# facebookresearch/videoseal

Measured on AMD Instinct MI355X. Metric: frames/sec embed+extract 256-bit @768x768, higher is better.
Workload: dtype f32 (2 x f16 operand split, 3 products on v_mfma_f32_32x32x16_f16, fp32 accumulate); 1 GPU; videoseal_1.0 256-bit, 32 frames 768x768 per GPU, image mode (embedder on every frame, full-res JND), embed + detect; card=videoseal_1.0, weights=random-init (seeded), no checkpoint offline, batch_per_gpu=32, mode=image

## Files before the change

videoseal_amd/csrc/net_ops.hip:

```cpp
#include <algorithm>
#include <cstdlib>
#include <cstring>

#include "conv_common.h"
#include "upconv_gather.h"

namespace {

__global__ __launch_bounds__(256) void layernorm_act_kernel(const float* __restrict__ x, int64_t rows, int C, int64_t ld,
                                                            const float* __restrict__ w, const float* __restrict__ b,
                                                            float eps, int act, float* __restrict__ out, int64_t out_ld) {
  const int lane = threadIdx.x & 63;
  const int64_t row = (int64_t)blockIdx.x * 4 + (threadIdx.x >> 6);
  if (row >= rows) return;
  const float* xr = x + row * ld;
  float s = 0.f;
  for (int c = lane; c < C; c += 64) s += xr[c];
  const float mean = wave_sum(s) / (float)C;
  float v = 0.f;
  for (int c = lane; c < C; c += 64) {
    const float dlt = xr[c] - mean;
    v += dlt * dlt;
  }
  const float var = wave_sum(v) / (float)C;
// ... 359 lines not shown
    for (int k = 0; k < LIN; ++k) {
      rin[k] = f32x4{0.f, 0.f, 0.f, 0.f};
      if (g_off[k] >= 0) rin[k] = *reinterpret_cast<const f32x4*>(xb + g_off[k] + c0);
    }
#pragma unroll
    for (int k = 0; k < LWT; ++k) {
      const int i = tid + k * NT;
      const int cg = i % N4, t = i / N4;
      if (i < NWT) rwt[k] = *reinterpret_cast<const f32x4*>((t < 49 ? wdw + (int64_t)t * ld : bdw) + c0 + cg * 4);
    }
  };
  const int nch = (int)ld / CCH;
  fetch(0);
  for (int ch = 0; ch < nch; ++ch) {
    const int c0 = ch * CCH;
#pragma unroll
    for (int k = 0; k < LIN; ++k)
      if (l_off[k] >= 0) *reinterpret_cast<f32x4*>(s_in + l_off[k]) = rin[k];
#pragma unroll
    for (int k = 0; k < LWT; ++k) {
      const int i = tid + k * NT;
      if (i < NWT) *reinterpret_cast<f32x4*>(s_w + (i / N4) * CCH + (i % N4) * 4) = rwt[k];
    }
    __syncthreads();
    if (ch + 1 < nch) fetch(c0 + CCH);
#ifdef VS_DWT_ABL
    if (!(VS_DWT_ABL & 2))
#endif
    for (int it = tid; it < ITEMS; it += NT) {
      const int cg = it % N4, rs = it / N4;
      const int sx = rs % SPR, r = rs / SPR;
      f32x4 acc[4];
      const f32x4 bv = *reinterpret_cast<const f32x4*>(s_w + 49 * CCH + cg * 4);
#pragma unroll
      for (int p = 0; p < 4; ++p) acc[p] = bv;
#pragma unroll
      for (int ky = 0; ky < 7; ++ky) {
        const float* row = s_in + ((r + ky) * IW + sx * 4) * CP + cg * 4;
        f32x4 in[10];
#pragma unroll
        for (int j = 0; j < 10; ++j) in[j] = *reinterpret_cast<const f32x4*>(row + j * CP);
#pragma unroll
        for (int kx = 0; kx < 7; ++kx) {
          const f32x4 wv = *reinterpret_cast<const f32x4*>(s_w + (ky * 7 + kx) * CCH + cg * 4);
#pragma unroll
          for (int p = 0; p < 4; ++p) acc[p] += in[p + kx] * wv;
        }
      }
#pragma unroll
      for (int p = 0; p < 4; ++p) *reinterpret_cast<f32x4*>(s_out + (int64_t)(r * TW + sx * 4 + p) * (ld + 4) + c0 + cg * 4) = acc[p];
    }
    __syncthreads();
  }
#ifdef VS_DWT_ABL
  if (VS_DWT_ABL & 1) return;
#endif
  ln_rows_from_lds<NT>(s_out, (int)ld + 4, TH * TW, C, lnw, lnb, eps, (int)out_ld, [&](int p) -> float* {
    const int gy = y0 + p / TW, gx = x0 + p % TW;
    return (gy < H && gx < W) ? out + (((int64_t)b * H + gy) * W + gx) * out_ld : nullptr;
  }, pl, wb_sep ? s_wbs : (2 * C <= (TH + 6) * (TW + 6) * CP) ? s_in : nullptr, wb_sep != 0);
}

template <int TH, int TW, int CCH, int NT>
static int launch_dwconv_tiled(const float* x, int B, int H, int W, int C, int64_t ld, const float* wdw, const float* bdw, const float* lnw,
                               const float* lnb, float eps, float* out, int64_t out_ld, hipStream_t st, PlanesOut pl = PlanesOut{0, 0, 1.f, 0}) {
  size_t smem = sizeof(float) * ((size_t)(TH + 6) * (TW + 6) * (CCH + 4) + 50 * CCH + (size_t)TH * TW * (ld + 4));
  if (smem > 160 * 1024 || ld % CCH != 0 || (int64_t)H * W * ld >= (1ll << 31)) return VS_ERR_UNSUPPORTED;
  const int wb_sep = smem + 2 * sizeof(float) * (size_t)C <= 160 * 1024;
  if (wb_sep) smem += 2 * sizeof(float) * (size_t)C;
  auto kern = dwconv7_ln_tiled_kernel<TH, TW, CCH, NT>;
  static size_t attr_set = 0;
  if (smem > 64 * 1024 && smem > attr_set) {
    (void)hipFuncSetAttribute((const void*)kern, hipFuncAttributeMaxDynamicSharedMemorySize, 160 * 1024);
    attr_set = 160 * 1024;
  }
  const int tiles_x = (W + TW - 1) / TW, tiles_y = (H + TH - 1) / TH;
  const int64_t nblk = (int64_t)B * tiles_x * tiles_y;
  if (nblk >= (1 << 30)) return VS_ERR_UNSUPPORTED;
  hipLaunchKernelGGL(kern, dim3((unsigned)((nblk + 7) / 8 * 8)), dim3(NT), smem, st, x, H, W, C, ld, wdw, bdw, lnw, lnb, eps, out, out_ld,
                     tiles_x, tiles_y, (int)nblk, pl, wb_sep);
  return vs_launch_status();
}

constexpr int GRN_ROWS = 64;
__global__ __launch_bounds__(256) void grn_partial_kernel(const float* __restrict__ h, int HW, int C, int64_t ld,
                                                          float* __restrict__ partial, int B) {
  const int c = blockIdx.x * 256 + threadIdx.x;
  const int chunk = blockIdx.y, b = blockIdx.z;
  if (c >= C) return;
  const int r0 = chunk * GRN_ROWS, r1 = min(HW, r0 + GRN_ROWS);
  const float* p = h + ((int64_t)b * HW + r0) * ld + c;
  float s = 0.f;
  for (int r = r0; r < r1; ++r, p += ld) s += (*p) * (*p);
  partial[((int64_t)chunk * B + b) * C + c] = s;
}
template <int NB, int KB>
__global__ __launch_bounds__(1024) void grn_finish_kernel(const float* __restrict__ partial, int nchunk, int B, int C,
                                                          const float* __restrict__ gamma, float* __restrict__ scale,
                                                          int64_t sld, int frame_major) {
  __shared__ float grp[NB][4][256];
  __shared__ float red[256];
  const int b = blockIdx.x;
  const int cl = threadIdx.x & 255, kg = threadIdx.x >> 8;
  const int kper = (nchunk + 3) / 4;
  const int k0 = kg * kper, k1 = min(nchunk, k0 + kper);
  float local = 0.f;
  for (int cb0 = 0; cb0 < C; cb0 += 256 * NB) {
    float s[NB];
#pragma unroll
    for (int j = 0; j < NB; ++j) s[j] = 0.f;
    const int64_t kstride = frame_major ? (int64_t)C : (int64_t)B * C;
    const float* rowp = frame_major ? partial + ((int64_t)b * nchunk + k0) * C : partial + ((int64_t)k0 * B + b) * C;
    int k = k0;
    for (; k + KB <= k1; k += KB, rowp += KB * kstride) {
      float v[KB][NB];
#pragma unroll
      for (int q = 0; q < KB; ++q)
#pragma unroll
        for (int j = 0; j < NB; ++j) {
          const int c = cb0 + j * 256 + cl;
          v[q][j] = c < C ? rowp[q * kstride + c] : 0.f;
        }
#pragma unroll
      for (int q = 0; q < KB; ++q)
#pragma unroll
        for (int j = 0; j < NB; ++j) s[j] += v[q][j];
    }
    if constexpr (KB > 4) {
      for (; k + 4 <= k1; k += 4, rowp += 4 * kstride) {
        float v[4][NB];
#pragma unroll
        for (int q = 0; q < 4; ++q)
#pragma unroll
          for (int j = 0; j < NB; ++j) {
            const int c = cb0 + j * 256 + cl;
            v[q][j] = c < C ? rowp[q * kstride + c] : 0.f;
          }
#pragma unroll
        for (int q = 0; q < 4; ++q)
#pragma unroll
          for (int j = 0; j < NB; ++j) s[j] += v[q][j];
      }
    }
    for (; k < k1; ++k, rowp += kstride) {
#pragma unroll
      for (int j = 0; j < NB; ++j) {
        const int c = cb0 + j * 256 + cl;
        if (c < C) s[j] += rowp[c];
      }
    }
#pragma unroll
    for (int j = 0; j < NB; ++j) grp[j][kg][cl] = s[j];
    __syncthreads();
    if (kg == 0) {
#pragma unroll
      for (int j = 0; j < NB; ++j) {
        const int c = cb0 + j * 256 + cl;
        if (c < C) {
          const float gx = sqrtf(((grp[j][0][cl] + grp[j][1][cl]) + grp[j][2][cl]) + grp[j][3][cl]);
          scale[(int64_t)b * sld + c] = gx;
          local += gx;
        }
      }
    }
    __syncthreads();
  }
// ... 589 lines not shown
  const int qd = threadIdx.x & 3;
  const int64_t npix = (int64_t)B * Ho * Wo;
  const int64_t pix = (int64_t)blockIdx.x * 64 + (threadIdx.x >> 2);
  const bool live = pix < npix;
  const int64_t pc = live ? pix : npix - 1;
  const int ox = (int)(pc % Wo);
  const int64_t t = pc / Wo;
  const int oy = (int)(t % Ho);
  const int64_t b = t / Ho;
  const float* xp = x + ((b * H + (int64_t)oy * stride) * W + (int64_t)ox * stride) * 4;
  f32x4 acc[Q4];
#pragma unroll
  for (int j = 0; j < Q4; ++j) acc[j] = *reinterpret_cast<const f32x4*>(bias + qd * CQ + 4 * j);
#pragma unroll
  for (int ky = 0; ky < 4; ++ky) {
    f32x4 in[4];
#pragma unroll
    for (int kx = 0; kx < 4; ++kx) in[kx] = *reinterpret_cast<const f32x4*>(xp + ((int64_t)ky * W + kx) * 4);
#pragma unroll
    for (int kx = 0; kx < 4; ++kx)
#pragma unroll
      for (int c = 0; c < 3; ++c) {
        const float v = in[kx][c];
        const float* wr = s_w + (ky * 12 + kx * 3 + c) * CO + qd * CQ;
#pragma unroll
        for (int j = 0; j < Q4; ++j) {
          const f32x4 wv = *reinterpret_cast<const f32x4*>(wr + 4 * j);
#pragma unroll
          for (int e = 0; e < 4; ++e) acc[j][e] = __builtin_fmaf(v, wv[e], acc[j][e]);
        }
      }
  }
  float sm = 0.f;
#pragma unroll
  for (int j = 0; j < Q4; ++j)
#pragma unroll
    for (int e = 0; e < 4; ++e) sm += acc[j][e];
  sm += __shfl_xor(sm, 1, 64);
  sm += __shfl_xor(sm, 2, 64);
  const float mean = sm / (float)CO;
  float qv = 0.f;
#pragma unroll
  for (int j = 0; j < Q4; ++j)
#pragma unroll
    for (int e = 0; e < 4; ++e) { const float dlt = acc[j][e] - mean; qv += dlt * dlt; }
  qv += __shfl_xor(qv, 1, 64);
  qv += __shfl_xor(qv, 2, 64);
  const float den = sqrtf(qv / (float)CO + eps);
  if (!live) return;
  float* orow = out + pix * out_ld + qd * CQ;
#pragma unroll
  for (int j = 0; j < Q4; ++j) {
    const f32x4 wv = *reinterpret_cast<const f32x4*>(lnw + qd * CQ + 4 * j), bv = *reinterpret_cast<const f32x4*>(lnb + qd * CQ + 4 * j);
    f32x4 o;
#pragma unroll
    for (int e = 0; e < 4; ++e) o[e] = wv[e] * ((acc[j][e] - mean) / den) + bv[e];
    *reinterpret_cast<f32x4*>(orow + 4 * j) = o;
  }
}

extern "C" int vs_stem_conv_ln(const float* x, int B, int H, int W, int stride, const float* wt, const float* bias, const float* lnw, const float* lnb,
                               float eps, int CO, float* out, int64_t out_ld, void* stream) {
  VS_REQUIRE(x && wt && bias && lnw && lnb && out && B > 0 && H >= 4 && W >= 4 && (stride == 4 || stride == 2));
  if ((CO != 64 && CO != 96 && CO != 128) || out_ld != CO ||
      (((uintptr_t)x | (uintptr_t)wt | (uintptr_t)bias | (uintptr_t)lnw | (uintptr_t)lnb | (uintptr_t)out) & 15) != 0)
    return VS_ERR_UNSUPPORTED;
  const int Ho = (H - 4) / stride + 1, Wo = (W - 4) / stride + 1;
  const int64_t npix = (int64_t)B * Ho * Wo;
  if (npix >= (1LL << 31) * 16) return VS_ERR_UNSUPPORTED;
  const dim3 grid((unsigned)cdiv64(npix, 64));
  hipStream_t st = (hipStream_t)stream;
  if (CO == 96) hipLaunchKernelGGL(stem_conv_ln_kernel<96>, grid, dim3(256), 0, st, x, B, H, W, Ho, Wo, stride, wt, bias, lnw, lnb, eps, out, out_ld);
  else if (CO == 64) hipLaunchKernelGGL(stem_conv_ln_kernel<64>, grid, dim3(256), 0, st, x, B, H, W, Ho, Wo, stride, wt, bias, lnw, lnb, eps, out, out_ld);
  else hipLaunchKernelGGL(stem_conv_ln_kernel<128>, grid, dim3(256), 0, st, x, B, H, W, Ho, Wo, stride, wt, bias, lnw, lnb, eps, out, out_ld);
  return vs_launch_status();
}

static int dwconv7_ln_any(const float* x, int B, int H, int W, int C, int64_t ld, const float* wdw, const float* bdw,
                          const float* lnw, const float* lnb, float eps, float* out, int64_t out_ld, void* stream, PlanesOut pl) {
  VS_REQUIRE(x && wdw && bdw && lnw && lnb && out && B > 0 && H > 0 && W > 0 && C > 0);
  VS_REQUIRE(ld % 4 == 0 && ld >= C && (pl.cstride || (out_ld >= C && out_ld % 4 == 0)));
  const int force = vs_debug_get(VS_DBG_DWCONV) - 1;
  {
    const int64_t hw = (int64_t)H * W;
    int cfg = 0;
    if (force >= 0) cfg = force;
    else if (hw >= 4096) cfg = 5;
    else if (hw >= 1024) cfg = 3;
    else if (hw >= 256) cfg = 6;
    int rc = VS_ERR_UNSUPPORTED;
    if (cfg == 1) rc = launch_dwconv_tiled<8, 8, 48, 256>(x, B, H, W, C, ld, wdw, bdw, lnw, lnb, eps, out, out_ld, (hipStream_t)stream, pl);
    else if (cfg == 2) rc = launch_dwconv_tiled<4, 8, 64, 128>(x, B, H, W, C, ld, wdw, bdw, lnw, lnb, eps, out, out_ld, (hipStream_t)stream, pl);
    else if (cfg == 3) rc = launch_dwconv_tiled<8, 16, 32, 256>(x, B, H, W, C, ld, wdw, bdw, lnw, lnb, eps, out, out_ld, (hipStream_t)stream, pl);
    else if (cfg == 4) rc = launch_dwconv_tiled<4, 16, 64, 256>(x, B, H, W, C, ld, wdw, bdw, lnw, lnb, eps, out, out_ld, (hipStream_t)stream, pl);
    else if (cfg == 5) rc = launch_dwconv_tiled<4, 16, 48, 256>(x, B, H, W, C, ld, wdw, bdw, lnw, lnb, eps, out, out_ld, (hipStream_t)stream, pl);
    else if (cfg == 6) rc = launch_dwconv_tiled<4, 8, 128, 256>(x, B, H, W, C, ld, wdw, bdw, lnw, lnb, eps, out, out_ld, (hipStream_t)stream, pl);
    else if (cfg == 7) rc = launch_dwconv_tiled<4, 4, 128, 128>(x, B, H, W, C, ld, wdw, bdw, lnw, lnb, eps, out, out_ld, (hipStream_t)stream, pl);
    else if (cfg == 8) rc = launch_dwconv_tiled<4, 4, 64, 128>(x, B, H, W, C, ld, wdw, bdw, lnw, lnb, eps, out, out_ld, (hipStream_t)stream, pl);
    else if (cfg == 9) rc = launch_dwconv_tiled<4, 4, 32, 128>(x, B, H, W, C, ld, wdw, bdw, lnw, lnb, eps, out, out_ld, (hipStream_t)stream, pl);
    else if (cfg == 10) rc = launch_dwconv_tiled<2, 8, 64, 128>(x, B, H, W, C, ld, wdw, bdw, lnw, lnb, eps, out, out_ld, (hipStream_t)stream, pl);
    if (rc == VS_ERR_UNSUPPORTED && force < 0 && cfg == 3)
      rc = launch_dwconv_tiled<4, 16, 48, 256>(x, B, H, W, C, ld, wdw, bdw, lnw, lnb, eps, out, out_ld, (hipStream_t)stream, pl);
    if (rc != VS_ERR_UNSUPPORTED) return rc;
  }
  const int C4 = (int)(ld / 4);
  int NS = 256 / C4;
  if (NS < 1) NS = 1;
  const int spr = (W + 3) / 4;
  const int dbg_rows = vs_debug_get(VS_DBG_DWCONV_ROWS);
  const bool two = dbg_rows ? dbg_rows == 2 : (NS == 1 && H >= 2 && (int64_t)B * ((H + 1) / 2) * spr >= vs_num_cus());
  const int R = two ? 2 : 1;
  const int64_t nstrips = (int64_t)B * ((H + R - 1) / R) * spr;
  const size_t smem = ((size_t)NS * 4 * R * (ld + 4) + 2 * (size_t)C) * sizeof(float);
  if (smem > 160 * 1024) return VS_ERR_UNSUPPORTED;
  if (two) {
    if (smem > 64 * 1024)
      (void)hipFuncSetAttribute((const void*)dwconv7_ln_kernel<2>, hipFuncAttributeMaxDynamicSharedMemorySize, (int)smem);
    hipLaunchKernelGGL(dwconv7_ln_kernel<2>, dim3((unsigned)cdiv64(nstrips, NS)), dim3(256), smem, (hipStream_t)stream, x, B, H, W,
                       C, ld, wdw, bdw, lnw, lnb, eps, out, out_ld, NS, spr, nstrips, pl);
    return vs_launch_status();
  }
  if (smem > 64 * 1024)
    (void)hipFuncSetAttribute((const void*)dwconv7_ln_kernel<1>, hipFuncAttributeMaxDynamicSharedMemorySize, (int)smem);
  hipLaunchKernelGGL(dwconv7_ln_kernel<1>, dim3((unsigned)cdiv64(nstrips, NS)), dim3(256), smem, (hipStream_t)stream, x, B, H, W,
                     C, ld, wdw, bdw, lnw, lnb, eps, out, out_ld, NS, spr, nstrips, pl);
  return vs_launch_status();
}

extern "C" int vs_dwconv7_ln(const float* x, int B, int H, int W, int C, int64_t ld, const float* wdw, const float* bdw,
                             const float* lnw, const float* lnb, float eps, float* out, int64_t out_ld, void* stream) {
  return dwconv7_ln_any(x, B, H, W, C, ld, wdw, bdw, lnw, lnb, eps, out, out_ld, stream, PlanesOut{0, 0, 1.f, 0});
}
extern "C" int vs_dwconv7_ln_planes(const float* x, int B, int H, int W, int C, int64_t ld, const float* wdw, const float* bdw,
                                    const float* lnw, const float* lnb, float eps, float a_mul, int planes_C, void* planes, void* stream) {
  VS_REQUIRE(planes && a_mul > 0.f && ((uintptr_t)planes & 15) == 0 && planes_C >= C && planes_C % 16 == 0);
  const int64_t rows = (int64_t)B * H * W, cstride = rows * 32;
  return dwconv7_ln_any(x, B, H, W, C, ld, wdw, bdw, lnw, lnb, eps, static_cast<float*>(planes), 8, stream,
                        PlanesOut{cstride, (int64_t)(planes_C / 16) * cstride, a_mul, planes_C});
}

extern "C" int vs_grn_scale(const float* h, int B, int HW, int C, int64_t ld, const float* gamma, float* partial,
                            float* scale, void* stream) {
  VS_REQUIRE(h && gamma && partial && scale && B > 0 && HW > 0 && C > 0 && ld >= C);
  const int nchunk = (HW + GRN_ROWS - 1) / GRN_ROWS;
  hipLaunchKernelGGL(grn_partial_kernel, dim3((unsigned)((C + 255) / 256), (unsigned)nchunk, (unsigned)B), dim3(256), 0,
                     (hipStream_t)stream, h, HW, C, ld, partial, B);
  if (C <= 512) hipLaunchKernelGGL((grn_finish_kernel<2, 16>), dim3((unsigned)B), dim3(1024), 0, (hipStream_t)stream, partial, nchunk, B, C, gamma,
                     scale, ld, 0);
  else if (C <= 1024) hipLaunchKernelGGL((grn_finish_kernel<4, 8>), dim3((unsigned)B), dim3(1024), 0, (hipStream_t)stream, partial, nchunk, B, C, gamma,
                     scale, ld, 0);
  else hipLaunchKernelGGL((grn_finish_kernel<8, 4>), dim3((unsigned)B), dim3(1024), 0, (hipStream_t)stream, partial, nchunk, B, C, gamma,
                     scale, ld, 0);
  return vs_launch_status();
}

__global__ __launch_bounds__(256) void grn_apply_kernel(float* __restrict__ h, int64_t rows, int HW, int C, int64_t ld,
                                                        const float* __restrict__ scale, int64_t sld, const float* __restrict__ beta) {
  const int C4 = (C + 3) >> 2;
  const int64_t idx = (int64_t)blockIdx.x * 256 + threadIdx.x;
  if (idx >= rows * C4) return;
  const int64_t m = idx / C4;
  const int c = (int)(idx - m * C4) * 4;
  const int b = (int)(m / HW);
  f32x4 v = *reinterpret_cast<f32x4*>(h + m * ld + c);
  const f32x4 s = *reinterpret_cast<const f32x4*>(scale + (int64_t)b * sld + c);
  const f32x4 sh = *reinterpret_cast<const f32x4*>(beta + c);
  const f32x4 o = v * s + sh;
#pragma unroll
  for (int e = 0; e < 4; ++e) v[e] = c + e < C ? o[e] : v[e];
  *reinterpret_cast<f32x4*>(h + m * ld + c) = v;
}

extern "C" int vs_grn_apply(float* h, int B, int HW, int C, int64_t ld, const float* scale, int64_t scale_ld, const float* beta,
                            void* stream) {
  VS_REQUIRE(h && scale && beta && B > 0 && HW > 0 && C > 0 && ld >= C && (ld & 3) == 0 && (scale_ld & 3) == 0 && scale_ld >= ((C + 3) & ~3));
  const int64_t rows = (int64_t)B * HW, items = rows * ((C + 3) >> 2);
  hipLaunchKernelGGL(grn_apply_kernel, dim3((unsigned)cdiv64(items, 256)), dim3(256), 0, (hipStream_t)stream, h, rows, HW, C, ld, scale,
                     scale_ld, beta);
  return vs_launch_status();
}

extern "C" int vs_grn_scale_from_partials(const float* partial, int B, int HW, int C, const float* gamma, float* scale,
                                          int64_t scale_ld, void* stream) {
  VS_REQUIRE(partial && gamma && scale && B > 0 && HW > 0 && HW % 32 == 0 && C > 0 && scale_ld >= C);
  if (C <= 512) hipLaunchKernelGGL((grn_finish_kernel<2, 16>), dim3((unsigned)B), dim3(1024), 0, (hipStream_t)stream, partial, HW / 32, B, C, gamma,
// ... 239 lines not shown
```

videoseal_amd/csrc/vs_common.h:

```cpp
#pragma once
#include <hip/hip_runtime.h>
#include <stdint.h>
#include <stdlib.h>
#include <string.h>

#include "videoseal_hip.h"

typedef float f32x4 __attribute__((ext_vector_type(4)));
typedef float f32x16 __attribute__((ext_vector_type(16)));

#define VS_REQUIRE(cond)                  \
  do {                                    \
    if (!(cond)) return VS_ERR_BAD_ARG;   \
  } while (0)

static inline int vs_launch_status() { return hipGetLastError() == hipSuccess ? VS_OK : VS_ERR_LAUNCH; }

static inline int64_t cdiv64(int64_t a, int64_t b) { return (a + b - 1) / b; }

static inline vs_yuv420_surface_t vs_nv12_surface(const void* base, int H, int64_t pitch, int64_t frame_stride) {
  vs_yuv420_surface_t s{};
  unsigned char* p = static_cast<unsigned char*>(const_cast<void*>(base));
  s.plane[0] = p;
  s.plane[1] = p + (int64_t)H * pitch;
  s.pitch[0] = s.pitch[1] = pitch;
  s.frame_stride[0] = s.frame_stride[1] = frame_stride;
  s.depth = 8;
  return s;
}

#define VS_DBG_ANY (-0x7fffffff - 1)
#define VS_DBG_KEYS(X)                                                                                                                              \
  X(RESIZE_FORM, "VIDEOSEAL_RESIZE", "tile=1", 0, 1, "vs_resize_pre(_nv12): 1 = the 32 x 8 tile kernel")                                            \
  X(RESIZE_STRIP, "VS_RESIZE_STRIP", nullptr, 0, 2, "vs_resize_pre(_nv12): strip height in output rows (the variable from 2, the key from 1)")      \
  X(TAIL_STRIP, "VS_TAIL_STRIP", nullptr, 0, 4, "vs_embed_tail(_nv12): strip height in rows, rounded up to 4 (from 4)")                             \
  X(JPEG_FORM, "VIDEOSEAL_JPEG", "scalar=1", 0, 1, "JPEG round trip: 1 = the one-pixel-per-lane kernels")                                           \
  X(CROP_RESIZE_FORM, "VIDEOSEAL_CROP_RESIZE", "tile=1", 0, 1, "Crop -> Resize -> colour: 1 = the 32 x 8 tile kernel")                              \
  X(TO_PLANES_FORM, nullptr, nullptr, 0, 1, "vs_to_planes_affine: 1 = one row per wave")                                                            \
  X(DWCONV_ROWS, "VS_DWCONV_ROWS", nullptr, 0, VS_DBG_ANY, "one-row depthwise kernel: 2 = two output rows per strip, any other value = one")        \
  X(LN_FORM, "VIDEOSEAL_LN", "wave=1", 0, 1, "vs_layernorm_act: 1 = one wave per row")                                                              \
  X(SPLITK_EPI, "VS_SPLITK_EPI", "s*=1", 0, 1, "K-slice epilogue: 1 = the first kernel, one load in flight per thread (VS_SPLITK_EPI=scalar)")      \
  X(UPCONV_FORM, nullptr, nullptr, 0, 1, "vs_upconv_gather_ln and phase 3 of vs_upconv_fused: 1 = per-pixel gather instead of 2 x 2 blocks")        \
  X(TAIL_FORM, "VIDEOSEAL_TAIL", "v1=1,sep=2,keep=3", 0, 1, "vs_embed_tail: the numbers of vs_tail_desc_t::variant (which overrides it per call)")  \
  X(VIT_ATTN, "VS_VIT_ATTN", "valu=1", 0, 1, "vs_vit_attention: 1 = the vector kernel on the matrix-core shapes too")                               \
  X(WGRAD, "VS_WGRAD", "mfma=1,fma=2", 0, 1, "vs_gemm_wgrad: 1 = the fp32 matrix-core kernel, 2 = the fp32 vector kernel, everywhere")              \
  X(DWCONV, "VS_DWCONV", nullptr, 1, 1, "depthwise 7 x 7 + LayerNorm: 1 + configuration (1 = the one-row kernel, 2.. = tiled; VS_DWCONV=0 -> 1)")    \
  X(GEMM_GRID, "VS_GEMM_GRID", nullptr, 0, 1, "wave-specialised 1 x 1 GEMM: workgroups of the persistent grid instead of one per CU")               \
  X(GEMM_PL_RASTER, "VS_GEMM_PL_RASTER", "0*=1", 0, 1, "planes GEMMs: 1 = row-major tile order instead of the XCD-grouped one (the variable: 0)")    \
  X(CNX_PIPE, "VS_CNX_PIPE", nullptr, 1, 1, "fused ConvNeXt block: 1 = the serial cnx_block_kernel (VS_CNX_PIPE=0), any other value = the pipeline") \
  X(CNX_ABL, "VS_CNX_ABL", nullptr, 0, VS_DBG_ANY, "fused ConvNeXt block: ablation bits (builds with VS_CNX_ABLATION only)")                        \
  X(UPCONV_ABL, "VS_UPCONV_ABL", nullptr, 0, VS_DBG_ANY, "vs_upconv_fused: ablation bits")                                                          \
  X(STEM_FUSED, "VIDEOSEAL_STEM_FUSED", "1*=1", 0, 1, "vs_model_detect: 1 = stem conv + LayerNorm in one kernel")                                   \
  X(ARITH, "VIDEOSEAL_CONV", "f16x2=2,bf16x3=3", 0, 2, "default vs_conv_desc_t::arith of the model-level entry points")
#define VS_DBG_ENUM(name, env, words, bias, min, doc) VS_DBG_##name,
enum { VS_DBG_KEYS(VS_DBG_ENUM) VS_DBG_COUNT };
#undef VS_DBG_ENUM
static_assert(VS_DBG_RESIZE_FORM == 0 && VS_DBG_UPCONV_FORM == 9 && VS_DBG_ARITH == 20 && VS_DBG_COUNT == 21, "development switch keys keep their numbers");

#define VS_DEFAULT_ARITH 2
static inline int vs_default_arith() {
  const int a = vs_debug_get(VS_DBG_ARITH);
  return a == 2 || a == 3 ? a : VS_DEFAULT_ARITH;
}

static inline int vs_max_lds_bytes() {
  static const int n = [] {
    int dev = 0, v = 0;
    if (hipGetDevice(&dev) != hipSuccess || hipDeviceGetAttribute(&v, hipDeviceAttributeMaxSharedMemoryPerBlock, dev) != hipSuccess || v <= 0) v = 64 * 1024;
    return v;
  }();
  return n;
}

static inline int vs_num_cus() {
  static const int n = [] {
    int dev = 0, v = 0;
    if (hipGetDevice(&dev) != hipSuccess || hipDeviceGetAttribute(&v, hipDeviceAttributeMultiprocessorCount, dev) != hipSuccess || v <= 0) v = 256;
    return v;
  }();
  return n;
}

__device__ __forceinline__ float vs_erfc_sqrt2(float a) {
  const float u = fminf(a, 5.65685424949238f);
  float q = 5.128553084e-07f;
  q = __builtin_fmaf(q, u, -9.560153558e-06f);
  q = __builtin_fmaf(q, u, 7.497344632e-05f);
  q = __builtin_fmaf(q, u, -2.843466646e-04f);
  q = __builtin_fmaf(q, u, 1.498938855e-05f);
  q = __builtin_fmaf(q, u, 6.931120995e-03f);
  q = __builtin_fmaf(q, u, -5.243476480e-02f);
  q = __builtin_fmaf(q, u, -4.592214525e-01f);
  q = __builtin_fmaf(q, u, -1.151104212e+00f);
  return __builtin_amdgcn_exp2f(q * u);
}
__device__ __forceinline__ float vs_gelu(float v) {
  const float a = fabsf(v);
  const float e = vs_erfc_sqrt2(a);
  return fmaxf(v, 0.f) - (0.5f * a) * e;
}
typedef float vs_f32x2 __attribute__((ext_vector_type(2)));
__device__ __forceinline__ vs_f32x2 vs_gelu2(const vs_f32x2 v) {
#pragma clang fp contract(off)
  const vs_f32x2 a = {fabsf(v[0]), fabsf(v[1])};
  const vs_f32x2 u = {fminf(a[0], 5.65685424949238f), fminf(a[1], 5.65685424949238f)};
  vs_f32x2 q = {5.128553084e-07f, 5.128553084e-07f};
  q = __builtin_elementwise_fma(q, u, vs_f32x2{-9.560153558e-06f, -9.560153558e-06f});
  q = __builtin_elementwise_fma(q, u, vs_f32x2{7.497344632e-05f, 7.497344632e-05f});
  q = __builtin_elementwise_fma(q, u, vs_f32x2{-2.843466646e-04f, -2.843466646e-04f});
  q = __builtin_elementwise_fma(q, u, vs_f32x2{1.498938855e-05f, 1.498938855e-05f});
  q = __builtin_elementwise_fma(q, u, vs_f32x2{6.931120995e-03f, 6.931120995e-03f});
  q = __builtin_elementwise_fma(q, u, vs_f32x2{-5.243476480e-02f, -5.243476480e-02f});
  q = __builtin_elementwise_fma(q, u, vs_f32x2{-4.592214525e-01f, -4.592214525e-01f});
  q = __builtin_elementwise_fma(q, u, vs_f32x2{-1.151104212e+00f, -1.151104212e+00f});
  const vs_f32x2 t = q * u;
  const vs_f32x2 e = {__builtin_amdgcn_exp2f(t[0]), __builtin_amdgcn_exp2f(t[1])};
  const vs_f32x2 m = {fmaxf(v[0], 0.f), fmaxf(v[1], 0.f)};
  return __builtin_elementwise_fma(a * -0.5f, e, m);
}
__device__ __forceinline__ float vs_gelu_grad(float v) {
  const float e = vs_erfc_sqrt2(fabsf(v));
  const float Phi = v >= 0.f ? 1.f - 0.5f * e : 0.5f * e;
  return Phi + v * (0.3989422804014327f * __expf(-0.5f * v * v));
}

__device__ __forceinline__ float vs_relu(float v) { return v <= 0.f ? 0.f : v; }

__device__ __forceinline__ float vs_apply_act(float v, int act) {
  switch (act) {
// ... 14 lines not shown
```

Measured before the change: 4453 frames/s.

## Add register-accumulating depthwise 7x7+LayerNorm kernel for high-res stages

Adds a new depthwise 7x7 conv + LayerNorm kernel that holds all channel chunks' accumulators in registers, so LayerNorm statistics are computed without re-reading the conv output from LDS. The kernel optionally prefetches the next channel chunk from global memory into registers while the current one computes, and processes two output rows per thread with a sliding weight window. It is selected by default for the large-resolution ld=96 and mid-resolution ld=192 stages, with the old LDS-tiled configs kept as fallback. The cost is heavy register use and a more complex LayerNorm reduction through shared memory partials.

Result: no change. 4474 frames/s (median of 6 runs) (+0.5%).

```diff
diff --git a/videoseal_amd/csrc/net_ops.hip b/videoseal_amd/csrc/net_ops.hip
--- a/videoseal_amd/csrc/net_ops.hip
+++ b/videoseal_amd/csrc/net_ops.hip
@@ -465,6 +465,295 @@
   return vs_launch_status();
 }
 
+template <int TH, int TW, int CCH, int NCH, int R, int NT, bool PF, int WPS>
+__global__ __launch_bounds__(NT, WPS) void dwconv7_ln_regs_kernel(const float* __restrict__ x, int H, int W, int C, int64_t ld,
+                                                                  const float* __restrict__ wdw, const float* __restrict__ bdw,
+                                                                  const float* __restrict__ lnw, const float* __restrict__ lnb,
+                                                                  float eps, float* __restrict__ out, int64_t out_ld, int tiles_x,
+                                                                  int tiles_y, int nblk, PlanesOut pl) {
+  constexpr int IH = TH + 6, IW = TW + 6, CP = CCH + 4, SPR = TW / 4, N4 = CCH / 4;
+  constexpr int NIN = IH * IW * N4, NWT = 50 * N4;
+  constexpr int LIN = (NIN + NT - 1) / NT, LWT = (NWT + NT - 1) / NT;
+  static_assert((TH / R) * SPR * N4 == NT && TH % R == 0 && TW % 4 == 0 && N4 % 4 == 0 && (R == 1 || R == 2), "one work item per thread");
+  static_assert(2 * TH * TW * (N4 + 1) <= IH * IW * CP && TH * TW <= NT, "the LayerNorm partials lie over the halo tile");
+  extern __shared__ __attribute__((aligned(16))) float smem[];
+  float* const s_in = smem;
+  float* const s_w = s_in + IH * IW * CP;
+  float* const s_wb = s_w + 50 * CCH;
+  const int tid = threadIdx.x;
+  const int per = (nblk + 7) >> 3;
+  const int vb = (blockIdx.x & 7) * per + (blockIdx.x >> 3);
+  if (vb >= nblk) return;
+  for (int i = tid; i < (int)ld; i += NT) {
+    s_wb[i] = i < C ? lnw[i] : 0.f;
+    s_wb[ld + i] = i < C ? lnb[i] : 0.f;
+  }
+  const int tx = vb % tiles_x;
+  const int t1 = vb / tiles_x;
+  const int ty = t1 % tiles_y;
+  const int b = t1 / tiles_y;
+  const int y0 = ty * TH, x0 = tx * TW;
+  const float* xb = x + (int64_t)b * H * W * ld;
+  const int cg = tid % N4, rs = tid / N4;
+  const int sx = rs % SPR, r = rs / SPR;
+  const int nch = (int)ld / CCH;
+  f32x4 rin[LIN], rwt[LWT];
+  auto fetch = [&](int c0) __attribute__((always_inline)) {
+#pragma unroll
+    for (int k = 0; k < LIN; ++k) {
+      const int i = tid + k * NT;
+      const int g = i % N4, pp = i / N4;
+      const int px = pp % IW, py = pp / IW;
+      const int gy = y0 + py - 3, gx = x0 + px - 3;
+      rin[k] = f32x4{0.f, 0.f, 0.f, 0.f};
+      if (i < NIN && gy >= 0 && gy < H && gx >= 0 && gx < W) rin[k] = *reinterpret_cast<const f32x4*>(xb + ((int64_t)gy * W + gx) * ld + c0 + g * 4);
+    }
+#pragma unroll
+    for (int k = 0; k < LWT; ++k) {
+      const int i = tid + k * NT;
+      const int g = i % N4, t = i / N4;
+      if (i < NWT) rwt[k] = *reinterpret_cast<const f32x4*>((t < 49 ? wdw + (int64_t)t * ld : bdw) + c0 + g * 4);
+    }
+  };
+  auto commit = [&]() __attribute__((always_inline)) {
+#pragma unroll
+    for (int k = 0; k < LIN; ++k) {
+      const int i = tid + k * NT;
+      if (i < NIN) *reinterpret_cast<f32x4*>(s_in + (i / N4) * CP + (i % N4) * 4) = rin[k];
+    }
+#pragma unroll
+    for (int k = 0; k < LWT; ++k) {
+      const int i = tid + k * NT;
+      if (i < NWT) *reinterpret_cast<f32x4*>(s_w + (i / N4) * CCH + (i % N4) * 4) = rwt[k];
+    }
+  };
+  f32x4 acc[NCH][R][4];
+  if (PF) fetch(0);
+#pragma unroll
+  for (int ch = 0; ch < NCH; ++ch) {
+    if (ch < nch) {
+      if (!PF) fetch(ch * CCH);
+      commit();
+      __syncthreads();
+      if (PF && ch + 1 < nch) fetch((ch + 1) * CCH);
+      const f32x4 bv = *reinterpret_cast<const f32x4*>(s_w + 49 * CCH + cg * 4);
+#pragma unroll
+      for (int rr = 0; rr < R; ++rr)
+#pragma unroll
+        for (int p = 0; p < 4; ++p) acc[ch][rr][p] = bv;
+      f32x4 wprev[7];
+#pragma unroll
+      for (int kr = 0; kr < 6 + R; ++kr) {
+        const float* row = s_in + ((r * R + kr) * IW + sx * 4) * CP + cg * 4;
+        f32x4 in[10];
+#pragma unroll
+        for (int j = 0; j < 10; ++j) in[j] = *reinterpret_cast<const f32x4*>(row + j * CP);
+        f32x4 wcur[7];
+        if (kr < 7) {
+#pragma unroll
+          for (int kx = 0; kx < 7; ++kx) wcur[kx] = *reinterpret_cast<const f32x4*>(s_w + (kr * 7 + kx) * CCH + cg * 4);
+#pragma unroll
+          for (int kx = 0; kx < 7; ++kx)
+#pragma unroll
+            for (int p = 0; p < 4; ++p) acc[ch][0][p] += in[p + kx] * wcur[kx];
+        }
+        if (R == 2 && kr >= 1) {
+#pragma unroll
+          for (int kx = 0; kx < 7; ++kx)
+#pragma unroll
+            for (int p = 0; p < 4; ++p) acc[ch][R - 1][p] += in[p + kx] * wprev[kx];
+        }
+        if (R == 2 && kr < 7) {
+#pragma unroll
+          for (int kx = 0; kx < 7; ++kx) wprev[kx] = wcur[kx];
+        }
+      }
+      __syncthreads();
+    }
+  }
+  float* const s_p1 = s_in;
+  float* const s_p2 = s_in + TH * TW * N4;
+  float* const s_t = s_p2 + TH * TW * N4;
+  const float invC = 1.0f / (float)C;
+  const int O4 = pl.cstride ? pl.Cp >> 2 : (int)out_ld >> 2;
+  f32x4 gw[NCH], gb[NCH];
+#pragma unroll
+  for (int k = 0; k < NCH; ++k)
+    if (k < nch) {
+      gw[k] = *reinterpret_cast<const f32x4*>(s_wb + k * CCH + cg * 4);
+      gb[k] = *reinterpret_cast<const f32x4*>(s_wb + ld + k * CCH + cg * 4);
+    }
+  const int lp0 = r * R * TW + sx * 4;
+#pragma unroll
+  for (int rr = 0; rr < R; ++rr)
+#pragma unroll
+    for (int p = 0; p < 4; ++p) {
+      float s = 0.f;
+#pragma unroll
+      for (int k = 0; k < NCH; ++k)
+        if (k < nch) {
+          const int c = k * CCH + cg * 4;
+          const f32x4 v = acc[k][rr][p];
+          s += ((c < C ? v[0] : 0.f) + (c + 1 < C ? v[1] : 0.f)) + ((c + 2 < C ? v[2] : 0.f) + (c + 3 < C ? v[3] : 0.f));
+        }
+      s_p1[(lp0 + rr * TW + p) * N4 + cg] = s;
+    }
+  constexpr bool TWO = N4 >= 32;
+  auto totals = [&](const float* s_p, float* s_t, float (&tot)[R][4]) __attribute__((always_inline)) {
+    __syncthreads();
+    if (TWO) {
+      if (tid < TH * TW) {
+        float s = 0.f;
+#pragma unroll
+        for (int j = 0; j < N4 / 4; ++j) {
+          const f32x4 t = *reinterpret_cast<const f32x4*>(s_p + tid * N4 + 4 * j);
+          s += (t[0] + t[1]) + (t[2] + t[3]);
+        }
+        s_t[tid] = s;
+      }
+      __syncthreads();
+#pragma unroll
+      for (int rr = 0; rr < R; ++rr) {
+        const f32x4 t = *reinterpret_cast<const f32x4*>(s_t + lp0 + rr * TW);
+#pragma unroll
+        for (int p = 0; p < 4; ++p) tot[rr][p] = t[p];
+      }
+    } else {
+#pragma unroll
+      for (int rr = 0; rr < R; ++rr)
+#pragma unroll
+        for (int p = 0; p < 4; ++p) {
+          const float* pr = s_p + (lp0 + rr * TW + p) * N4;
+          float s = 0.f;
+#pragma unroll
+          for (int j = 0; j < N4 / 4; ++j) {
+            const f32x4 t = *reinterpret_cast<const f32x4*>(pr + 4 * j);
+            s += (t[0] + t[1]) + (t[2] + t[3]);
+          }
+          tot[rr][p] = s;
+        }
+    }
+  };
+  float mean[R][4], var[R][4];
+  totals(s_p1, s_t, mean);
+#pragma unroll
+  for (int rr = 0; rr < R; ++rr)
+#pragma unroll
+    for (int p = 0; p < 4; ++p) {
+      mean[rr][p] *= invC;
+      float q = 0.f;
+#pragma unroll
+      for (int k = 0; k < NCH; ++k)
+        if (k < nch) {
+#pragma unroll
+          for (int e = 0; e < 4; ++e) {
+            const float dl = (k * CCH + cg * 4 + e < C) ? acc[k][rr][p][e] - mean[rr][p] : 0.f;
+            q += dl * dl;
+          }
+        }
+      s_p2[(lp0 + rr * TW + p) * N4 + cg] = q;
+    }
+  totals(s_p2, s_t + TH * TW, var);
+  float rden[R][4];
+#pragma unroll
+  for (int rr = 0; rr < R; ++rr)
+#pragma unroll
+    for (int p = 0; p < 4; ++p) rden[rr][p] = 1.0f / sqrtf(var[rr][p] * invC + eps);
+  auto norm = [&](int k, int rr, int p) __attribute__((always_inline)) -> f32x4 {
+    f32x4 o = {0.f, 0.f, 0.f, 0.f};
+#pragma unroll
+    for (int e = 0; e < 4; ++e)
+      if (k * CCH + cg * 4 + e < C) o[e] = gw[k][e] * ((acc[k][rr][p][e] - mean[rr][p]) * rden[rr][p]) + gb[k][e];
+    return o;
+  };
+  if (pl.cstride) {
+    const int j = tid & 3;
+    auto pick = [&](const vsconv::u32x2 (&a)[4], int i) __attribute__((always_inline)) -> vsconv::u32x2 {
+      const vsconv::u32x2 lo2 = (i & 1) ? a[1] : a[0], hi2 = (i & 1) ? a[3] : a[2];
+      return (i & 2) ? hi2 : lo2;
+    };
+    auto xchg = [&](vsconv::u32x2 v, int t) __attribute__((always_inline)) -> vsconv::u32x2 {
+      return vsconv::u32x2{(unsigned)__shfl_xor((int)v[0], t, 64), (unsigned)__shfl_xor((int)v[1], t, 64)};
+    };
+#pragma unroll
+    for (int rr = 0; rr < R; ++rr) {
+      const int gy = y0 + r * R + rr, gx = x0 + sx * 4 + j;
+      const bool ok = gy < H && gx < W;
+      char* const prow = reinterpret_cast<char*>(out) + (((int64_t)b * H + gy) * W + gx) * 32;
+#pragma unroll
+      for (int k = 0; k < NCH; ++k) {
+        const int c4 = k * N4 + cg;
+        if (k < nch && c4 < O4) {
+          vsconv::u32x2 hi[4], lo[4], th[4], tl[4];
+#pragma unroll
+          for (int p = 0; p < 4; ++p) vsconv::split4h(norm(k, rr, p), pl.a_mul, hi[p], lo[p]);
+          th[0] = pick(hi, j); tl[0] = pick(lo, j);
+#pragma unroll
+          for (int t = 1; t < 4; ++t) { th[t] = xchg(pick(hi, j ^ t), t); tl[t] = xchg(pick(lo, j ^ t), t); }
+          if (ok) {
+            char* dst = prow + (int64_t)(c4 >> 2) * pl.cstride;
+            const bool odd = j & 1;
+            const vsconv::u32x4 ha = {(odd ? th[1] : th[0])[0], (odd ? th[1] : th[0])[1], (odd ? th[0] : th[1])[0], (odd ? th[0] : th[1])[1]};
+            const vsconv::u32x4 hb = {(odd ? th[3] : th[2])[0], (odd ? th[3] : th[2])[1], (odd ? th[2] : th[3])[0], (odd ? th[2] : th[3])[1]};
+            const vsconv::u32x4 la = {(odd ? tl[1] : tl[0])[0], (odd ? tl[1] : tl[0])[1], (odd ? tl[0] : tl[1])[0], (odd ? tl[0] : tl[1])[1]};
+            const vsconv::u32x4 lb = {(odd ? tl[3] : tl[2])[0], (odd ? tl[3] : tl[2])[1], (odd ? tl[2] : tl[3])[0], (odd ? tl[2] : tl[3])[1]};
+            const int oa = (j >> 1) * 16, ob = 16 - oa;
+            *reinterpret_cast<vsconv::u32x4*>(dst + oa) = ha;
+            *reinterpret_cast<vsconv::u32x4*>(dst + ob) = hb;
+            *reinterpret_cast<vsconv::u32x4*>(dst + pl.pstride + oa) = la;
+            *reinterpret_cast<vsconv::u32x4*>(dst + pl.pstride + ob) = lb;
+          }
+        }
+      }
+      if (ok)
+        for (int c4 = nch * N4 + (cg & ~3); c4 < O4; c4 += N4) {
+          char* dst = prow + (int64_t)(c4 >> 2) * pl.cstride;
+          const vsconv::u32x4 z = {0u, 0u, 0u, 0u};
+          *reinterpret_cast<vsconv::u32x4*>(dst) = z;
+          *reinterpret_cast<vsconv::u32x4*>(dst + 16) = z;
+          *reinterpret_cast<vsconv::u32x4*>(dst + pl.pstride) = z;
+          *reinterpret_cast<vsconv::u32x4*>(dst + pl.pstride + 16) = z;
+        }
+    }
+    return;
+  }
+#pragma unroll
+  for (int rr = 0; rr < R; ++rr)
+#pragma unroll
+    for (int p = 0; p < 4; ++p) {
+      const int gy = y0 + r * R + rr, gx = x0 + sx * 4 + p;
+      if (gy >= H || gx >= W) continue;
+      float* orow = out + (((int64_t)b * H + gy) * W + gx) * out_ld;
+#pragma unroll
+      for (int k = 0; k < NCH; ++k) {
+        const int c4 = k * N4 + cg;
+        if (k < nch && c4 < O4) *reinterpret_cast<f32x4*>(orow + 4 * c4) = norm(k, rr, p);
+      }
+      for (int c4 = nch * N4 + cg; c4 < O4; c4 += N4) *reinterpret_cast<f32x4*>(orow + 4 * c4) = f32x4{0.f, 0.f, 0.f, 0.f};
+    }
+}
+
+template <int TH, int TW, int CCH, int NCH, int R, int NT, bool PF, int WPS>
+static int launch_dwconv_regs(const float* x, int B, int H, int W, int C, int64_t ld, const float* wdw, const float* bdw, const float* lnw,
+                              const float* lnb, float eps, float* out, int64_t out_ld, hipStream_t st, PlanesOut pl) {
+  constexpr size_t tile = sizeof(float) * ((size_t)(TH + 6) * (TW + 6) * (CCH + 4) + 50 * CCH);
+  static_assert(tile + 2 * sizeof(float) * NCH * CCH <= 160 * 1024, "tile beyond the LDS of a CU");
+  if (ld % CCH != 0 || ld / CCH > NCH || (int64_t)H * W * ld >= (1ll << 31)) return VS_ERR_UNSUPPORTED;
+  const size_t smem = tile + 2 * sizeof(float) * (size_t)ld;
+  auto kern = dwconv7_ln_regs_kernel<TH, TW, CCH, NCH, R, NT, PF, WPS>;
+  static bool attr_set = false;
+  if (smem > 64 * 1024 && !attr_set) {
+    (void)hipFuncSetAttribute((const void*)kern, hipFuncAttributeMaxDynamicSharedMemorySize, 160 * 1024);
+    attr_set = true;
+  }
+  const int tiles_x = (W + TW - 1) / TW, tiles_y = (H + TH - 1) / TH;
+  const int64_t nblk = (int64_t)B * tiles_x * tiles_y;
+  if (nblk >= (1 << 30)) return VS_ERR_UNSUPPORTED;
+  hipLaunchKernelGGL(kern, dim3((unsigned)((nblk + 7) / 8 * 8)), dim3(NT), smem, st, x, H, W, C, ld, wdw, bdw, lnw, lnb, eps, out, out_ld,
+                     tiles_x, tiles_y, (int)nblk, pl);
+  return vs_launch_status();
+}
+
 constexpr int GRN_ROWS = 64;
 __global__ __launch_bounds__(256) void grn_partial_kernel(const float* __restrict__ h, int HW, int C, int64_t ld,
                                                           float* __restrict__ partial, int B) {
@@ -1220,25 +1509,35 @@
   VS_REQUIRE(ld % 4 == 0 && ld >= C && (pl.cstride || (out_ld >= C && out_ld % 4 == 0)));
   const int force = vs_debug_get(VS_DBG_DWCONV) - 1;
   {
+    auto run = [&](int cfg) -> int {
+      if (cfg == 1) return launch_dwconv_tiled<8, 8, 48, 256>(x, B, H, W, C, ld, wdw, bdw, lnw, lnb, eps, out, out_ld, (hipStream_t)stream, pl);
+      if (cfg == 2) return launch_dwconv_tiled<4, 8, 64, 128>(x, B, H, W, C, ld, wdw, bdw, lnw, lnb, eps, out, out_ld, (hipStream_t)stream, pl);
+      if (cfg == 3) return launch_dwconv_tiled<8, 16, 32, 256>(x, B, H, W, C, ld, wdw, bdw, lnw, lnb, eps, out, out_ld, (hipStream_t)stream, pl);
+      if (cfg == 4) return launch_dwconv_tiled<4, 16, 64, 256>(x, B, H, W, C, ld, wdw, bdw, lnw, lnb, eps, out, out_ld, (hipStream_t)stream, pl);
+      if (cfg == 5) return launch_dwconv_tiled<4, 16, 48, 256>(x, B, H, W, C, ld, wdw, bdw, lnw, lnb, eps, out, out_ld, (hipStream_t)stream, pl);
+      if (cfg == 6) return launch_dwconv_tiled<4, 8, 128, 256>(x, B, H, W, C, ld, wdw, bdw, lnw, lnb, eps, out, out_ld, (hipStream_t)stream, pl);
+      if (cfg == 7) return launch_dwconv_tiled<4, 4, 128, 128>(x, B, H, W, C, ld, wdw, bdw, lnw, lnb, eps, out, out_ld, (hipStream_t)stream, pl);
+      if (cfg == 8) return launch_dwconv_tiled<4, 4, 64, 128>(x, B, H, W, C, ld, wdw, bdw, lnw, lnb, eps, out, out_ld, (hipStream_t)stream, pl);
+      if (cfg == 9) return launch_dwconv_tiled<4, 4, 32, 128>(x, B, H, W, C, ld, wdw, bdw, lnw, lnb, eps, out, out_ld, (hipStream_t)stream, pl);
+      if (cfg == 10) return launch_dwconv_tiled<2, 8, 64, 128>(x, B, H, W, C, ld, wdw, bdw, lnw, lnb, eps, out, out_ld, (hipStream_t)stream, pl);
+      if (cfg == 11) return launch_dwconv_regs<16, 16, 32, 3, 2, 256, false, 2>(x, B, H, W, C, ld, wdw, bdw, lnw, lnb, eps, out, out_ld, (hipStream_t)stream, pl);
+      if (cfg == 12) return launch_dwconv_regs<8, 16, 64, 3, 1, 512, true, 2>(x, B, H, W, C, ld, wdw, bdw, lnw, lnb, eps, out, out_ld, (hipStream_t)stream, pl);
+      if (cfg == 13) return launch_dwconv_regs<4, 8, 192, 2, 1, 384, true, 2>(x, B, H, W, C, ld, wdw, bdw, lnw, lnb, eps, out, out_ld, (hipStream_t)stream, pl);
+      if (cfg == 14) return launch_dwconv_regs<8, 16, 32, 3, 1, 256, false, 3>(x, B, H, W, C, ld, wdw, bdw, lnw, lnb, eps, out, out_ld, (hipStream_t)stream, pl);
+      return VS_ERR_UNSUPPORTED;
+    };
     const int64_t hw = (int64_t)H * W;
-    int cfg = 0;
-    if (force >= 0) cfg = force;
-    else if (hw >= 4096) cfg = 5;
-    else if (hw >= 1024) cfg = 3;
-    else if (hw >= 256) cfg = 6;
     int rc = VS_ERR_UNSUPPORTED;
-    if (cfg == 1) rc = launch_dwconv_tiled<8, 8, 48, 256>(x, B, H, W, C, ld, wdw, bdw, lnw, lnb, eps, out, out_ld, (hipStream_t)stream, pl);
-    else if (cfg == 2) rc = launch_dwconv_tiled<4, 8, 64, 128>(x, B, H, W, C, ld, wdw, bdw, lnw, lnb, eps, out, out_ld, (hipStream_t)stream, pl);
-    else if (cfg == 3) rc = launch_dwconv_tiled<8, 16, 32, 256>(x, B, H, W, C, ld, wdw, bdw, lnw, lnb, eps, out, out_ld, (hipStream_t)stream, pl);
-    else if (cfg == 4) rc = launch_dwconv_tiled<4, 16, 64, 256>(x, B, H, W, C, ld, wdw, bdw, lnw, lnb, eps, out, out_ld, (hipStream_t)stream, pl);
-    else if (cfg == 5) rc = launch_dwconv_tiled<4, 16, 48, 256>(x, B, H, W, C, ld, wdw, bdw, lnw, lnb, eps, out, out_ld, (hipStream_t)stream, pl);
-    else if (cfg == 6) rc = launch_dwconv_tiled<4, 8, 128, 256>(x, B, H, W, C, ld, wdw, bdw, lnw, lnb, eps, out, out_ld, (hipStream_t)stream, pl);
-    else if (cfg == 7) rc = launch_dwconv_tiled<4, 4, 128, 128>(x, B, H, W, C, ld, wdw, bdw, lnw, lnb, eps, out, out_ld, (hipStream_t)stream, pl);
-    else if (cfg == 8) rc = launch_dwconv_tiled<4, 4, 64, 128>(x, B, H, W, C, ld, wdw, bdw, lnw, lnb, eps, out, out_ld, (hipStream_t)stream, pl);
-    else if (cfg == 9) rc = launch_dwconv_tiled<4, 4, 32, 128>(x, B, H, W, C, ld, wdw, bdw, lnw, lnb, eps, out, out_ld, (hipStream_t)stream, pl);
-    else if (cfg == 10) rc = launch_dwconv_tiled<2, 8, 64, 128>(x, B, H, W, C, ld, wdw, bdw, lnw, lnb, eps, out, out_ld, (hipStream_t)stream, pl);
-    if (rc == VS_ERR_UNSUPPORTED && force < 0 && cfg == 3)
-      rc = launch_dwconv_tiled<4, 16, 48, 256>(x, B, H, W, C, ld, wdw, bdw, lnw, lnb, eps, out, out_ld, (hipStream_t)stream, pl);
+    if (force >= 0) rc = run(force);
+    else {
+      if (hw >= 4096 && ld == 96) rc = run(11);
+      else if (hw >= 1024 && hw < 4096 && ld == 192) rc = run(12);
+      if (rc == VS_ERR_UNSUPPORTED) {
+        const int cfg = hw >= 4096 ? 5 : hw >= 1024 ? 3 : hw >= 256 ? 6 : 0;
+        rc = run(cfg);
+        if (rc == VS_ERR_UNSUPPORTED && cfg == 3) rc = run(5);
+      }
+    }
     if (rc != VS_ERR_UNSUPPORTED) return rc;
   }
   const int C4 = (int)(ld / 4);
diff --git a/videoseal_amd/csrc/vs_common.h b/videoseal_amd/csrc/vs_common.h
--- a/videoseal_amd/csrc/vs_common.h
+++ b/videoseal_amd/csrc/vs_common.h
@@ -44,7 +44,7 @@
   X(TAIL_FORM, "VIDEOSEAL_TAIL", "v1=1,sep=2,keep=3", 0, 1, "vs_embed_tail: the numbers of vs_tail_desc_t::variant (which overrides it per call)")  \
   X(VIT_ATTN, "VS_VIT_ATTN", "valu=1", 0, 1, "vs_vit_attention: 1 = the vector kernel on the matrix-core shapes too")                               \
   X(WGRAD, "VS_WGRAD", "mfma=1,fma=2", 0, 1, "vs_gemm_wgrad: 1 = the fp32 matrix-core kernel, 2 = the fp32 vector kernel, everywhere")              \
-  X(DWCONV, "VS_DWCONV", nullptr, 1, 1, "depthwise 7 x 7 + LayerNorm: 1 + configuration (1 = the one-row kernel, 2.. = tiled; VS_DWCONV=0 -> 1)")    \
+  X(DWCONV, "VS_DWCONV", nullptr, 1, 1, "depthwise 7 x 7 + LayerNorm: 1 + configuration (1 = the one-row kernel, 2-11 = LDS-parked tiles, 12-15 = register-parked; VS_DWCONV=0 -> 1)")    \
   X(GEMM_GRID, "VS_GEMM_GRID", nullptr, 0, 1, "wave-specialised 1 x 1 GEMM: workgroups of the persistent grid instead of one per CU")               \
   X(GEMM_PL_RASTER, "VS_GEMM_PL_RASTER", "0*=1", 0, 1, "planes GEMMs: 1 = row-major tile order instead of the XCD-grouped one (the variable: 0)")    \
   X(CNX_PIPE, "VS_CNX_PIPE", nullptr, 1, 1, "fused ConvNeXt block: 1 = the serial cnx_block_kernel (VS_CNX_PIPE=0), any other value = the pipeline") \
```
